# RicoFio/disentangle_mlp

Measured on AMD Instinct MI355X. Metric: celeba64_betavaegan_train_images_per_sec, higher is better.
Workload: dtype fp32-equivalent (fp16x3 split of fp32 operands on the f16 MFMA, fp32 accumulate, every convolution and the Linear layers with >= 2^20 weights (vg_gemm_nt_f16x3); the small Linear layers (vendor GEMMs), BatchNorm, losses, Adam in fp32)

## Files before the change

disentangle_mlp_amd/csrc/common.hpp:

```cpp
#pragma once
#include <hip/hip_runtime.h>
#include <stdint.h>

typedef float f32x16 __attribute__((ext_vector_type(16)));
typedef float f32x4 __attribute__((ext_vector_type(4)));

#define VG_WAVE 64

#ifdef VG_TUNING
#define VG_KNOB(type, name, value) type name = value
#else
#define VG_KNOB(type, name, value) constexpr type name = value
#endif

#define VG_CHECK_LAUNCH()                         \
  do {                                            \
    hipError_t e__ = hipGetLastError();           \
    if (e__ != hipSuccess) return (int)e__;       \
  } while (0)

__device__ __forceinline__ f32x16 mfma32(float a, float b, f32x16 c) {
  return __builtin_amdgcn_mfma_f32_32x32x2f32(a, b, c, 0, 0, 0);
}

__device__ __forceinline__ int acc_row(int r, int lane) {
  return (r & 3) + 8 * (r >> 2) + 4 * (lane >> 5);
}

__device__ __forceinline__ float act_slope(float v, float slope) { return v * (v > 0.f ? 1.f : slope); }

typedef __attribute__((ext_vector_type(8))) __bf16 bf16x8;
typedef __attribute__((ext_vector_type(8))) _Float16 f16x8;

#define VG_PLANES_F16_FLAG 0x100

constexpr int VG_PACK_SPARE = 6;
constexpr size_t vg_pack_trailer_units(int nsteps, int planes, int CoutP) {
  return (size_t)(nsteps + VG_PACK_SPARE) * planes * 2 * CoutP;
}

constexpr int VG_STATS_SLOT_DEPTH = 16;

__device__ __forceinline__ unsigned f16_bound_exp(float amax) {
  const unsigned e = (__float_as_uint(amax) >> 23) & 0xffu;
  return min(max(e, 15u), 254u);
}
__device__ __forceinline__ float f16_scale_of(float amax) { return __uint_as_float((268u - f16_bound_exp(amax)) << 23); }
__device__ __forceinline__ float f16_unscale_of(float amax) { return __uint_as_float((f16_bound_exp(amax) - 14u) << 23); }

template <int NP, bool F16>
__device__ __forceinline__ void split_planes16(float* v, f32x4* out) {
  if constexpr (F16) {
    static_assert(NP == 2, "fp16 planes: hi + lo");
    typedef float f32x2 __attribute__((ext_vector_type(2)));
    typedef _Float16 f16x2 __attribute__((ext_vector_type(2)));
    f16x2 hi[4], lo[4];
#pragma unroll
    for (int j = 0; j < 4; ++j) {
      const f32x2 v2 = {v[2 * j], v[2 * j + 1]};
      const f16x2 h = __builtin_convertvector(v2, f16x2);
      hi[j] = h;
      lo[j] = __builtin_convertvector(v2 - __builtin_convertvector(h, f32x2), f16x2);
    }
    struct P4 { f16x2 q[4]; };
    out[0] = __builtin_bit_cast(f32x4, P4{{hi[0], hi[1], hi[2], hi[3]}});
    out[1] = __builtin_bit_cast(f32x4, P4{{lo[0], lo[1], lo[2], lo[3]}});
  } else {
#pragma unroll
    for (int p = 0; p < NP; ++p) {
      bf16x8 q;
#pragma unroll
      for (int j = 0; j < 8; ++j) {
        const __bf16 h = (__bf16)v[j];
        q[j] = h;
        v[j] -= (float)h;
      }
      out[p] = __builtin_bit_cast(f32x4, q);
    }
  }
}

template <bool F16>
__device__ __forceinline__ f32x16 mfma_split16(bf16x8 a, bf16x8 b, f32x16 c) {
  if constexpr (F16)
    return __builtin_amdgcn_mfma_f32_32x32x16_f16(__builtin_bit_cast(f16x8, a), __builtin_bit_cast(f16x8, b), c, 0, 0, 0);
  else
    return __builtin_amdgcn_mfma_f32_32x32x16_bf16(a, b, c, 0, 0, 0);
}

template <typename T>
__device__ __forceinline__ T wave_sum(T v) {
#pragma unroll
  for (int o = 32; o > 0; o >>= 1) v += __shfl_down(v, o, 64);
  return v;
}

template <typename T>
__device__ __forceinline__ T wave_allsum(T v) {
#pragma unroll
  for (int o = 32; o > 0; o >>= 1) v += __shfl_xor(v, o, 64);
  return v;
}

template <int NT, typename T>
__device__ __forceinline__ T block_sum(T v, T* red) {
  v = wave_sum(v);
  const int lane = threadIdx.x & 63, wid = threadIdx.x >> 6;
  __syncthreads();
  if (lane == 0) red[wid] = v;
  __syncthreads();
  T t = 0;
  if (threadIdx.x == 0) {
#pragma unroll
    for (int i = 0; i < NT / 64; ++i) t += red[i];
  }
  return t;
}

__device__ __forceinline__ unsigned abs_bits(float v) { return __float_as_uint(v) & 0x7fffffffu; }

template <int NT>
__device__ __forceinline__ void block_amax_atomic(unsigned m, unsigned* out) {
  __shared__ unsigned amax_red[NT / 64];
#pragma unroll
  for (int o = 32; o > 0; o >>= 1) m = max(m, (unsigned)__shfl_xor((int)m, o, 64));
  const int lane = threadIdx.x & 63, wid = threadIdx.x >> 6;
  if (lane == 0) amax_red[wid] = m;
  __syncthreads();
  if (threadIdx.x == 0) {
#pragma unroll
    for (int i = 1; i < NT / 64; ++i) m = max(m, amax_red[i]);
    if (m > __hip_atomic_load(out, __ATOMIC_RELAXED, __HIP_MEMORY_SCOPE_AGENT)) atomicMax(out, m);
  }
}

__host__ __device__ constexpr int cdiv(int a, int b) { return (a + b - 1) / b; }

int vg_internal_wgrad_reduce(const float* slabs, float* dw, int n, int splits, hipStream_t st, int accumulate = 0);
size_t vg_internal_ring_workspace_bytes(int mode, int B, int Cin, int H, int W, int Cout, int planes);
size_t vg_internal_ring_stats_floats(int mode, int B, int Cin, int H, int W, int Cout, int planes);
int vg_internal_ring_conv(int mode, const float* x, const void* packed, const float* bias, float* y, int B, int Cin, int H,
                          int W, int Cout, int planes, void* workspace, size_t workspace_bytes, const float* in_scale,
                          const float* in_shift, int in_act, float* stats, size_t stats_floats, const float* in_amax,
                          hipStream_t st);
#ifdef VG_TUNING
void vg_internal_ring_set_variant(int v);
void vg_internal_wx_set_th(int th);
#endif
int vg_internal_convT_s1_thin(const float* x, const float* w, const float* bias, float* y, int B, int Cin, int H,
                              int W, int Cout, hipStream_t st);
```

disentangle_mlp_amd/csrc/wgrad_bf16split.hip:

```cpp
#include <algorithm>
#include <vector>

#include "common.hpp"
#include "vaegan_hip.h"

namespace {

constexpr int WTW = 8, WCIT = 5;

struct WXArgs {
  const float* x;
  int B;
  const float* in_scale;
  const float* in_shift;
  float in_slope;
  const bf16x8* gp;
  float* ws;
  int Cin, H, W, Cout, CoP, OH, OW;
  int mtiles, ntiles, tiles_w, tiles_hw, chunks;
  int units, upw;
  unsigned short order[256];
  const float* x_amax;
};

template <int NP, bool F16>
__global__ __launch_bounds__(256) void relayout_gy_kernel(const float* __restrict__ gy, bf16x8* __restrict__ gp,
                                                         int B, int Co, int CoP, int P, const float* __restrict__ g_scale,
                                                         const float* __restrict__ g_shift, float g_slope,
                                                         const float* __restrict__ g_amax) {
  __shared__ float tile[8][32][33];
  const float gsc16 = F16 ? f16_scale_of(*g_amax) : 1.f;
  const int tid = threadIdx.x;
  const int p0 = blockIdx.x * 32, co0 = blockIdx.y * 32;
  const int bg = blockIdx.z >> 1, kb = blockIdx.z & 1;
  if ((P & 3) == 0 && p0 + 32 <= P && ((uintptr_t)gy & 15) == 0) {
    const int co = co0 + (tid >> 3), q4 = (tid & 7) * 4;
    const float sc = (g_scale && co < Co) ? g_scale[co] : 1.f, sh = (g_scale && co < Co) ? g_shift[co] : 0.f;
    f32x4 v[8];
#pragma unroll
    for (int j = 0; j < 8; ++j) {
      const int b = bg * 16 + kb * 8 + j;
      const float* src = gy + ((size_t)min(b, B - 1) * Co + min(co, Co - 1)) * P + p0 + q4;
      v[j] = *reinterpret_cast<const f32x4*>(src);
    }
#pragma unroll
    for (int j = 0; j < 8; ++j) {
      const bool ok = (bg * 16 + kb * 8 + j) < B && co < Co;
#pragma unroll
      for (int e = 0; e < 4; ++e) {
        float t = v[j][e];
        if (g_scale) {
          t = fmaf(t, sc, sh);
          t = act_slope(t, g_slope);
        }
        tile[j][tid >> 3][q4 + e] = ok ? t : 0.f;
      }
    }
  } else {
    const int r = tid >> 5, pl = tid & 31;
#pragma unroll
    for (int j = 0; j < 8; ++j) {
      const int b = bg * 16 + kb * 8 + j;
#pragma unroll
      for (int rr = 0; rr < 4; ++rr) {
        const int co = co0 + r + 8 * rr;
        float v = 0.f;
        if (b < B && co < Co && p0 + pl < P) {
          v = gy[((size_t)b * Co + co) * P + p0 + pl];
          if (g_scale) {
            v = fmaf(v, g_scale[co], g_shift[co]);
            v = act_slope(v, g_slope);
          }
        }
        tile[j][r + 8 * rr][pl] = v;
      }
    }
  }
  __syncthreads();
  const int cc = tid & 31;
#pragma unroll
  for (int k = 0; k < 4; ++k) {
    const int pp = (tid >> 5) + 8 * k;
    if (p0 + pp >= P) continue;
    float v[8];
#pragma unroll
    for (int j = 0; j < 8; ++j) v[j] = F16 ? tile[j][cc][pp] * gsc16 : tile[j][cc][pp];
    f32x4 pl[NP];
    split_planes16<NP, F16>(v, pl);
#pragma unroll
    for (int p = 0; p < NP; ++p)
      gp[((((size_t)bg * P + p0 + pp) * NP + p) * 2 + kb) * CoP + co0 + cc] = __builtin_bit_cast(bf16x8, pl[p]);
  }
}

constexpr int W8NT = 512;

template <int S_, int NP_, int WCO_, int TH_, bool F16_ = false>
struct W8 {
  static constexpr int S = S_, NP = NP_, WCO = WCO_, WN = 8 / WCO_, FP = 4 / WN, TCO = 32 * WCO_;
  static constexpr bool F16 = F16_;
  static constexpr int TH = TH_, NPIX = TH_ * WTW;
  static constexpr int PD = (FP <= 2) ? 7 : 3;
  static constexpr int PH = S * (TH - 1) + 5, PW = S * (WTW - 1) + 5;
  static constexpr int ROWU = PW + ((5 - PW % 16) + 16) % 16;
  static constexpr int CIU = PH * ROWU + ((9 - (PH * ROWU) % 16) + 16) % 16;
  static constexpr int KBU = WCIT * CIU;
  static constexpr int BUFU = 2 * NP * KBU;
  static constexpr int NUNIT = 2 * WCIT * PH * PW;
  static constexpr int NQ = cdiv(NUNIT, W8NT);
  static constexpr int STEP = TH, ST0 = NPIX / 4;
  static_assert(ST0 + 2 * NQ * STEP <= NPIX, "store schedule");
  static_assert(NPIX % (PD + 1) == 0, "gy ring");
  static_assert(2 * BUFU * 16 <= 160 * 1024, "LDS");
};

template <class C>
__global__ __launch_bounds__(W8NT, 2) void conv5x5_wgrad_split8_kernel(WXArgs A) {
  constexpr int S = C::S, PH = C::PH, PW = C::PW, ROWU = C::ROWU, CIU = C::CIU, KBU = C::KBU, NQ = C::NQ;
  constexpr int NP = C::NP, FP = C::FP, BUFU = C::BUFU, PD = C::PD;
  constexpr bool F16 = C::F16;
  __shared__ f32x4 lds[2 * BUFU];
  const float x_scale = F16 ? f16_scale_of(*A.x_amax) : 1.f;
  const int tid = threadIdx.x, lane = tid & 63;
  const int wid = __builtin_amdgcn_readfirstlane(tid >> 6);
  const int kb = lane >> 5, l32 = lane & 31;
  const int wm = wid % C::WCO, wn = wid / C::WCO;
  const int grp = wid >> 2;
  const int wg = A.order[blockIdx.x];
  const int u_begin = wg * A.upw, u_end = min(u_begin + A.upw, A.units);
  const int Cin = A.Cin, Cout = A.Cout, H = A.H, W = A.W, OW = A.OW, CoP = A.CoP;
  const int HW = H * W, P = A.OH * A.OW;
  int m0 = 0, ci0 = 0;

  int desc[NQ];
#pragma unroll
  for (int q = 0; q < NQ; ++q) {
    const int e = tid + q * W8NT;
    const int col = e % PW;
    int t = e / PW;
    const int r = t % PH;
    t /= PH;
    const int ci = t % WCIT, kbs = min(t / WCIT, 1);
    desc[q] = r | (col << 4) | (ci << 9) | (kbs << 12) | ((e < C::NUNIT ? 1 : 0) << 13);
  }
  static_assert(PH <= 16 && PW <= 32 && WCIT <= 8, "descriptor fields");

  auto chunk_pos = [&](int chunk, int& bg, int& oh, int& ow0) {
    bg = chunk / A.tiles_hw;
    const int sp = chunk % A.tiles_hw;
    oh = (sp / A.tiles_w) * C::TH;
    ow0 = (sp % A.tiles_w) * WTW;
  };
  float preg[NQ][8], psc[NQ], psh[NQ];
  unsigned pvalid = 0;
  const size_t chw = (size_t)Cin * HW;
  auto load_patch = [&](int chunk) {
    int bg, oh, ow0;
    chunk_pos(chunk, bg, oh, ow0);
    const int ih0 = S * oh - 2, iw0 = S * ow0 - 2;
    pvalid = 0;
#pragma unroll
    for (int q = 0; q < NQ; ++q) {
      const int d = desc[q];
      const int ih = ih0 + (d & 15), iw = iw0 + ((d >> 4) & 31);
      const int ci = (d >> 9) & 7, kbs = (d >> 12) & 1;
      const bool ok = ih >= 0 && ih < H && iw >= 0 && iw < W && (ci0 + ci) < Cin;
      pvalid |= ok ? (1u << q) : 0u;
      const int cc = min(ci0 + ci, Cin - 1);
      const unsigned off = (unsigned)(cc * HW + min(max(ih, 0), H - 1) * W + min(max(iw, 0), W - 1));
      psc[q] = A.in_scale ? A.in_scale[cc] : 1.f;
      psh[q] = A.in_scale ? A.in_shift[cc] : 0.f;
      const int b0 = bg * 16 + kbs * 8;
#pragma unroll
      for (int j = 0; j < 8; ++j) {
        const float* xb = A.x + (size_t)min(b0 + j, A.B - 1) * chw;
        preg[q][j] = xb[off];
      }
    }
  };
  auto store_unit = [&](int q, int buf, int chunk) {
    const int bgrp = chunk / A.tiles_hw;
    const int d = desc[q];
    const int kbs = (d >> 12) & 1;
    const bool live = (pvalid >> q) & 1u;
    float v[8];
#pragma unroll
    for (int j = 0; j < 8; ++j) {
      float t = fmaf(preg[q][j], psc[q], psh[q]);
      t = act_slope(t, A.in_slope);
      t = F16 ? t * x_scale : t;
      v[j] = (live && (bgrp * 16 + kbs * 8 + j) < A.B) ? t : 0.f;
    }
    f32x4 pl[NP];
    split_planes16<NP, F16>(v, pl);
    const int dst = buf * BUFU + kbs * KBU + ((d >> 9) & 7) * CIU + (d & 15) * ROWU + ((d >> 4) & 31);
    if (d >> 13) {
#pragma unroll
      for (int p = 0; p < NP; ++p) lds[dst + p * 2 * KBU] = pl[p];
    }
  };
  auto store_patch = [&](int buf, int chunk) {
#pragma unroll
    for (int q = 0; q < NQ; ++q) store_unit(q, buf, chunk);
  };
  static_assert(NQ <= 32, "validity mask");

  int base_b[FP];
#pragma unroll
  for (int f = 0; f < FP; ++f) {
    const int n = min((wn * FP + f) * 32 + l32, WCIT * 25 - 1);
    const int ci = n / 25, tap = n % 25;
    base_b[f] = kb * KBU + ci * CIU + (tap / 5) * ROWU + tap % 5;
  }
  const size_t gstep = (size_t)2 * NP * CoP;
  auto pix_off = [&](int k) -> size_t { return (size_t)(k >> 3) * OW + (k & 7); };

  const int u_split = (u_begin / A.chunks + 1) * A.chunks;
  const bool two = u_split < u_end && u_end <= u_split + A.chunks;
  int u = two ? u_split : u_begin, u_lim = u_end, pass = 0, t0 = 0;
  while (true) {
    if (u >= u_lim) {
      if (!two || pass) break;
      pass = 1;
      u = u_begin;
      u_lim = u_split;
      continue;
    }
    const int tile = u / A.chunks, c_begin = u - tile * A.chunks;
    const int c_end = min(A.chunks, c_begin + (u_lim - u));
    u += c_end - c_begin;
    m0 = (tile % A.mtiles) * C::TCO;
    ci0 = (tile / A.mtiles) * WCIT;
    const bf16x8* ga = A.gp + (size_t)kb * CoP + m0 + wm * 32 + l32;

    f32x16 acc[FP];
#pragma unroll
    for (int f = 0; f < FP; ++f)
#pragma unroll
      for (int r = 0; r < 16; ++r) acc[f][r] = 0.f;

    auto chunk_pix = [&](int chunk) -> size_t {
      int bg, oh, ow0;
      chunk_pos(min(chunk, c_end - 1), bg, oh, ow0);
      return (size_t)bg * P + (size_t)oh * OW + ow0;
    };
    bf16x8 av[PD + 1][NP];
    static_assert((PD == 3 || PD == 7) && WTW == 8, "ring indices below assume 4 or 8 sets, 8 pixels per row");
    auto load_a = [&](int set, size_t pix) {
#pragma unroll
      for (int pl = 0; pl < NP; ++pl) av[set][pl] = ga[pix * gstep + (size_t)pl * 2 * CoP];
    };
    const int nch = c_end - c_begin;
    int rot = ((t0 - c_begin) % A.upw + A.upw) % A.upw;
    rot = rot < nch ? rot : 0;
    t0 += nch;
    auto chunk_at = [&](int j) -> int {
      int i = min(j, nch - 1) + rot;
      i -= (i >= nch) ? nch : 0;
      return c_begin + i;
    };
    load_patch(chunk_at(0));
    store_patch(0, chunk_at(0));
    size_t pcur = chunk_pix(chunk_at(0));
#pragma unroll
    for (int t = 0; t < PD; ++t) load_a(t, pcur + pix_off(t));
    __syncthreads();
    for (int j = 0; j < nch; ++j) {
      const int chn = chunk_at(j + 1);
      const int buf = j & 1;
      const bool more = (j + 1) < nch;
      const size_t pnxt = chunk_pix(chn);
#pragma unroll
      for (int t = 0; t < C::NPIX; ++t) {
        load_a((t + PD) & PD, (t + PD < C::NPIX) ? pcur + pix_off(t + PD) : pnxt + pix_off(t + PD - C::NPIX));
        if (t == 0 && more) load_patch(chn);
        bf16x8 bv[FP][NP];
#pragma unroll
        for (int f = 0; f < FP; ++f)
#pragma unroll
          for (int pl = 0; pl < NP; ++pl)
            bv[f][pl] = __builtin_bit_cast(
                bf16x8, lds[buf * BUFU + base_b[f] + S * (t >> 3) * ROWU + S * (t & 7) + pl * 2 * KBU]);
#pragma unroll
        for (int sum = NP - 1; sum >= 0; --sum)
#pragma unroll
          for (int pa = sum; pa >= 0; --pa)
#pragma unroll
            for (int f = 0; f < FP; ++f) acc[f] = mfma_split16<F16>(av[t & PD][pa], bv[f][sum - pa], acc[f]);
        {
          const int rel = t - C::ST0;
          if (rel >= 0 && rel % C::STEP == 0 && rel / C::STEP < 2 * NQ) {
            const int q = (rel / C::STEP) % NQ, g = (rel / C::STEP) / NQ;
            if (more && grp == g) store_unit(q, buf ^ 1, chn);
          }
        }
      }
      __syncthreads();
      pcur = pnxt;
    }

    const int piece = wg - (int)(((long)tile * A.chunks) / A.upw);
    float* wsb = A.ws + (size_t)piece * Cout * Cin * 25;
#pragma unroll
    for (int f = 0; f < FP; ++f) {
      const int n = (wn * FP + f) * 32 + l32;
      const bool nok = n < WCIT * 25 && (ci0 + n / 25) < Cin;
#pragma unroll
      for (int r16 = 0; r16 < 16; ++r16) {
        const int co = m0 + wm * 32 + acc_row(r16, lane);
        if (nok && co < Cout) wsb[((size_t)co * Cin + ci0) * 25 + n] = acc[f][r16];
      }
    }
  }
}

__global__ __launch_bounds__(256) void wx_reduce_kernel(const float* __restrict__ slabs, float* __restrict__ dw, int Cin,
                                                       int tco, int mtiles, int chunks, int upw, unsigned n, int accumulate,
                                                       const float* __restrict__ x_amax, const float* __restrict__ gy_amax) {
  const unsigned e = blockIdx.x * 256u + threadIdx.x;
  if (e >= n) return;
  const float ux = x_amax ? f16_unscale_of(*x_amax) : 1.f, ug = gy_amax ? f16_unscale_of(*gy_amax) : 1.f;
  const int row = Cin * 25, co = e / row, ci = (e - co * row) / 25;
  const long tile = (long)(ci / WCIT) * mtiles + co / tco;
  const int first = (int)((tile * chunks) / upw), last = (int)(((tile + 1) * chunks - 1) / upw);
  const int cnt = last - first + 1;
  float sum = 0.f;
  int p = 0;
  for (; p + 4 <= cnt; p += 4) {
    float v[4];
#pragma unroll
    for (int k = 0; k < 4; ++k) v[k] = slabs[(size_t)(p + k) * n + e];
#pragma unroll
    for (int k = 0; k < 4; ++k) sum += v[k];
  }
  for (; p < cnt; ++p) sum += slabs[(size_t)p * n + e];
  dw[e] = sum * ux * ug + (accumulate ? dw[e] : 0.f);
}

struct XPlan {
  int BG, CoP, OH, OW, wco, th, mtiles, ntiles, tiles_w, tiles_hw, chunks, units, upw, wgs, pieces;
  size_t gp_bytes, slab_bytes;
};

VG_KNOB(int, g_wx_th, 0);

void plan_shares(XPlan& p, int th) {
  p.th = th;
  p.tiles_hw = p.tiles_w * (p.OH / th);
  p.chunks = p.BG * p.tiles_hw;
  p.units = p.mtiles * p.ntiles * p.chunks;
  p.upw = cdiv(p.units, 256);
  p.wgs = cdiv(p.units, p.upw);
}

bool make_xplan(int B, int Cin, int H, int W, int Cout, int S, int planes, XPlan& p) {
  p.OH = (H - 1) / S + 1;
  p.OW = (W - 1) / S + 1;
  if (p.OW % WTW) return false;
  p.BG = cdiv(B, 16);
  p.CoP = (Cout + 127) & ~127;
  p.wco = Cout > 128 ? 8 : 4;
  p.mtiles = cdiv(Cout, 32 * p.wco);
  p.ntiles = cdiv(Cin, WCIT);
  p.tiles_w = p.OW / WTW;
  if ((long)p.mtiles * p.ntiles * p.BG * p.tiles_w * p.OH > 0x3fffffffL) return false;
  int th = (p.OH % 2 == 0) ? 2 : 1;
  if (g_wx_th == 1 || (g_wx_th == 2 && p.OH % 2 == 0)) th = g_wx_th;
  plan_shares(p, th);
  p.pieces = 0;
  for (long t = 0; t < (long)p.mtiles * p.ntiles; ++t) {
    const int first = (int)((t * p.chunks) / p.upw), last = (int)(((t + 1) * p.chunks - 1) / p.upw);
    p.pieces = last - first + 1 > p.pieces ? last - first + 1 : p.pieces;
  }
  p.gp_bytes = (size_t)p.BG * p.OH * p.OW * 2 * planes * p.CoP * 16;
  p.slab_bytes = (size_t)p.pieces * Cout * Cin * 25 * sizeof(float);
  return true;
}

void make_order(const XPlan& p, unsigned short* order) {
  std::vector<int> idx(p.wgs);
  for (int w = 0; w < p.wgs; ++w) idx[w] = w;
  std::stable_sort(idx.begin(), idx.end(), [&](int a, int b) {
    return ((long)a * p.upw) % p.chunks < ((long)b * p.upw) % p.chunks;
  });
  int start[9];
  start[0] = 0;
  for (int k = 0; k < 8; ++k) start[k + 1] = start[k] + (p.wgs - k + 7) / 8;
  for (int b = 0; b < p.wgs; ++b) order[b] = (unsigned short)idx[start[b & 7] + (b >> 3)];
}

template <class C>
int launch_wx(const WXArgs& A, long grid, hipStream_t st) {
  hipLaunchKernelGGL(conv5x5_wgrad_split8_kernel<C>, dim3((unsigned)grid), dim3(W8NT), 0, st, A);
  VG_CHECK_LAUNCH();
  return 0;
}

template <int S, int NP, bool F16 = false>
int launch_wx_by_cout(const WXArgs& A, int wco, int th, long grid, hipStream_t st) {
  if (th == 2) return wco == 8 ? launch_wx<W8<S, NP, 8, 2, F16>>(A, grid, st) : launch_wx<W8<S, NP, 4, 2, F16>>(A, grid, st);
  return wco == 8 ? launch_wx<W8<S, NP, 8, 1, F16>>(A, grid, st) : launch_wx<W8<S, NP, 4, 1, F16>>(A, grid, st);
}

}

#ifdef VG_TUNING
void vg_internal_wx_set_th(int th) { g_wx_th = (th == 1 || th == 2) ? th : 0; }
#endif

extern "C" size_t vg_conv5x5_wgrad_bf16split_workspace_bytes(int B, int Cin, int H, int W, int Cout, int stride,
                                                          int planes) {
  if (B <= 0 || Cin <= 0 || Cout <= 0 || H <= 0 || W <= 0 || (stride != 1 && stride != 2)) return 0;
  if (planes != 2 && planes != 3 && planes != (VG_PLANES_F16_FLAG | 2)) return 0;
  XPlan p;
  if (!make_xplan(B, Cin, H, W, Cout, stride, planes & 0xff, p)) return 0;
  return p.gp_bytes + p.slab_bytes;
}

extern "C" int vg_conv5x5_wgrad_bf16split(const float* x, const float* gy, float* dw, int B, int Cin, int H, int W,
                                       int Cout, int stride, int planes, void* workspace, size_t workspace_bytes,
                                       const float* in_scale, const float* in_shift, int in_act, int affine_on_gy,
                                       const float* x_amax, const float* gy_amax, int accumulate, void* stream) {
  if (!x || !gy || !dw || B <= 0 || Cin <= 0 || Cout <= 0 || H <= 0 || W <= 0) return VG_ERR_BAD_ARG;
  const bool f16 = (planes & VG_PLANES_F16_FLAG) != 0;
  planes &= 0xff;
  if (f16 && (planes != 2 || !x_amax || !gy_amax)) return VG_ERR_BAD_ARG;
  if (!f16) x_amax = gy_amax = nullptr;
  if ((in_scale == nullptr) != (in_shift == nullptr) || in_act < VG_ACT_NONE || in_act > VG_ACT_LRELU) return VG_ERR_BAD_ARG;
  const float slope = (!in_scale || in_act == VG_ACT_NONE) ? 1.f : (in_act == VG_ACT_RELU ? 0.f : 0.2f);
  const float* gsc = affine_on_gy ? in_scale : nullptr;
  const float* gsh = affine_on_gy ? in_shift : nullptr;
  if (affine_on_gy) in_scale = in_shift = nullptr;
  if ((stride != 1 && stride != 2) || (planes != 2 && planes != 3)) return VG_ERR_BAD_ARG;
  XPlan p;
  if (!make_xplan(B, Cin, H, W, Cout, stride, planes, p)) return VG_ERR_BAD_ARG;
  if (!workspace || ((uintptr_t)workspace & 15) || workspace_bytes < p.gp_bytes + p.slab_bytes)
    return VG_ERR_WORKSPACE;
  hipStream_t st = (hipStream_t)stream;
  bf16x8* gp = (bf16x8*)workspace;
  float* slabs = (float*)((char*)workspace + p.gp_bytes);
  const int P = p.OH * p.OW;
  if ((size_t)Cin * H * W * 4 > 0xffffffffUL || p.BG * 2 > 65535 || p.CoP / 32 > 65535) return VG_ERR_BAD_ARG;
  const dim3 gg(cdiv(P, 32), p.CoP / 32, p.BG * 2);
  if (f16) hipLaunchKernelGGL((relayout_gy_kernel<2, true>), gg, dim3(256), 0, st, gy, gp, B, Cout, p.CoP, P, gsc, gsh, slope, gy_amax);
  else if (planes == 2) hipLaunchKernelGGL((relayout_gy_kernel<2, false>), gg, dim3(256), 0, st, gy, gp, B, Cout, p.CoP, P, gsc, gsh, slope, gy_amax);
  else hipLaunchKernelGGL((relayout_gy_kernel<3, false>), gg, dim3(256), 0, st, gy, gp, B, Cout, p.CoP, P, gsc, gsh, slope, gy_amax);
  VG_CHECK_LAUNCH();
  WXArgs A;
  A.x = x; A.B = B; A.gp = gp; A.ws = slabs; A.x_amax = x_amax;
  A.in_scale = in_scale; A.in_shift = in_shift;
  A.in_slope = in_scale ? slope : 1.f;
  A.Cin = Cin; A.H = H; A.W = W; A.Cout = Cout; A.CoP = p.CoP; A.OH = p.OH; A.OW = p.OW;
  A.mtiles = p.mtiles; A.ntiles = p.ntiles; A.tiles_w = p.tiles_w; A.tiles_hw = p.tiles_hw;
  A.chunks = p.chunks; A.units = p.units; A.upw = p.upw;
  make_order(p, A.order);
  const long grid = p.wgs;
  int rc;
  if (f16) rc = (stride == 2) ? launch_wx_by_cout<2, 2, true>(A, p.wco, p.th, grid, st) : launch_wx_by_cout<1, 2, true>(A, p.wco, p.th, grid, st);
  else if (planes == 2) rc = (stride == 2) ? launch_wx_by_cout<2, 2>(A, p.wco, p.th, grid, st) : launch_wx_by_cout<1, 2>(A, p.wco, p.th, grid, st);
  else rc = (stride == 2) ? launch_wx_by_cout<2, 3>(A, p.wco, p.th, grid, st) : launch_wx_by_cout<1, 3>(A, p.wco, p.th, grid, st);
  if (rc) return rc;
  const unsigned n = (unsigned)Cout * Cin * 25;
  hipLaunchKernelGGL(wx_reduce_kernel, dim3(cdiv(n, 256u)), dim3(256), 0, st, slabs, dw, Cin, 32 * p.wco, p.mtiles,
                     p.chunks, p.upw, n, accumulate ? 1 : 0, x_amax, gy_amax);
  VG_CHECK_LAUNCH();
  return 0;
}
```

Measured before the change: 9295.

## Switch weight-gradient conv kernel from 32x32x16 to 16x16x32 MFMA tiles

Rewrites the inner loop of the 5x5 weight-gradient kernel to use 16x16x32 MFMA instructions, with K of 32 spanning two output pixels (pixel pairs) instead of 32x32x16 over single pixels. Each wave now covers its 32 output channels with two 16-row groups and twice as many 16-wide column tiles. The gradient register ring, LDS B-operand addressing, store schedule and accumulator writeback are reworked to match, and B loads are batched in groups of HB. The aim is better MFMA throughput and fewer accumulator registers per instruction. In exchange it adds more A-operand loads per step and more complex LDS indexing.

```diff
diff --git a/disentangle_mlp_amd/csrc/common.hpp b/disentangle_mlp_amd/csrc/common.hpp
--- a/disentangle_mlp_amd/csrc/common.hpp
+++ b/disentangle_mlp_amd/csrc/common.hpp
@@ -88,6 +88,14 @@
     return __builtin_amdgcn_mfma_f32_32x32x16_bf16(a, b, c, 0, 0, 0);
 }
 
+template <bool F16>
+__device__ __forceinline__ f32x4 mfma_split16x32(bf16x8 a, bf16x8 b, f32x4 c) {
+  if constexpr (F16)
+    return __builtin_amdgcn_mfma_f32_16x16x32_f16(__builtin_bit_cast(f16x8, a), __builtin_bit_cast(f16x8, b), c, 0, 0, 0);
+  else
+    return __builtin_amdgcn_mfma_f32_16x16x32_bf16(a, b, c, 0, 0, 0);
+}
+
 template <typename T>
 __device__ __forceinline__ T wave_sum(T v) {
 #pragma unroll
diff --git a/disentangle_mlp_amd/csrc/wgrad_bf16split.hip b/disentangle_mlp_amd/csrc/wgrad_bf16split.hip
--- a/disentangle_mlp_amd/csrc/wgrad_bf16split.hip
+++ b/disentangle_mlp_amd/csrc/wgrad_bf16split.hip
@@ -99,18 +99,20 @@
 struct W8 {
   static constexpr int S = S_, NP = NP_, WCO = WCO_, WN = 8 / WCO_, FP = 4 / WN, TCO = 32 * WCO_;
   static constexpr bool F16 = F16_;
-  static constexpr int TH = TH_, NPIX = TH_ * WTW;
-  static constexpr int PD = (FP <= 2) ? 7 : 3;
+  static constexpr int TH = TH_, NPAIR = TH_ * WTW / 2;
+  static constexpr int PD = (FP <= 2) ? 3 : 1;
+  static constexpr int HB = (NP == 3) ? 2 : 4;
   static constexpr int PH = S * (TH - 1) + 5, PW = S * (WTW - 1) + 5;
   static constexpr int ROWU = PW + ((5 - PW % 16) + 16) % 16;
   static constexpr int CIU = PH * ROWU + ((9 - (PH * ROWU) % 16) + 16) % 16;
-  static constexpr int KBU = WCIT * CIU;
+  static constexpr int KBU = (WCIT * CIU + 15) & ~15;
   static constexpr int BUFU = 2 * NP * KBU;
   static constexpr int NUNIT = 2 * WCIT * PH * PW;
   static constexpr int NQ = cdiv(NUNIT, W8NT);
-  static constexpr int STEP = TH, ST0 = NPIX / 4;
-  static_assert(ST0 + 2 * NQ * STEP <= NPIX, "store schedule");
-  static_assert(NPIX % (PD + 1) == 0, "gy ring");
+  static constexpr int SPP = 2 / TH, ST0 = NPAIR / 4;
+  static_assert(TH == 1 || TH == 2, "store slots per pair");
+  static_assert(ST0 + cdiv(2 * NQ, SPP) <= NPAIR, "store schedule");
+  static_assert(NPAIR % (PD + 1) == 0, "gy ring");
   static_assert(2 * BUFU * 16 <= 160 * 1024, "LDS");
 };
 
@@ -123,7 +125,7 @@
   const float x_scale = F16 ? f16_scale_of(*A.x_amax) : 1.f;
   const int tid = threadIdx.x, lane = tid & 63;
   const int wid = __builtin_amdgcn_readfirstlane(tid >> 6);
-  const int kb = lane >> 5, l32 = lane & 31;
+  const int kb = (lane >> 4) & 1, pq = lane >> 5, l16 = lane & 15;
   const int wm = wid % C::WCO, wn = wid / C::WCO;
   const int grp = wid >> 2;
   const int wg = A.order[blockIdx.x];
@@ -205,15 +207,15 @@
   };
   static_assert(NQ <= 32, "validity mask");
 
-  int base_b[FP];
-#pragma unroll
-  for (int f = 0; f < FP; ++f) {
-    const int n = min((wn * FP + f) * 32 + l32, WCIT * 25 - 1);
+  int base_b[2 * FP];
+#pragma unroll
+  for (int h = 0; h < 2 * FP; ++h) {
+    const int n = min((wn * 2 * FP + h) * 16 + l16, WCIT * 25 - 1);
     const int ci = n / 25, tap = n % 25;
-    base_b[f] = kb * KBU + ci * CIU + (tap / 5) * ROWU + tap % 5;
+    base_b[h] = kb * KBU + ci * CIU + (tap / 5) * ROWU + tap % 5 + S * pq;
   }
   const size_t gstep = (size_t)2 * NP * CoP;
-  auto pix_off = [&](int k) -> size_t { return (size_t)(k >> 3) * OW + (k & 7); };
+  auto pix_off = [&](int k) -> size_t { return (size_t)(k >> 2) * OW + 2 * (k & 3); };
 
   const int u_split = (u_begin / A.chunks + 1) * A.chunks;
   const bool two = u_split < u_end && u_end <= u_split + A.chunks;
@@ -231,24 +233,26 @@
     u += c_end - c_begin;
     m0 = (tile % A.mtiles) * C::TCO;
     ci0 = (tile / A.mtiles) * WCIT;
-    const bf16x8* ga = A.gp + (size_t)kb * CoP + m0 + wm * 32 + l32;
-
-    f32x16 acc[FP];
-#pragma unroll
-    for (int f = 0; f < FP; ++f)
-#pragma unroll
-      for (int r = 0; r < 16; ++r) acc[f][r] = 0.f;
+    const bf16x8* ga = A.gp + (size_t)pq * gstep + (size_t)kb * CoP + m0 + wm * 32 + l16;
+
+    f32x4 acc[2][2 * FP];
+#pragma unroll
+    for (int g = 0; g < 2; ++g)
+#pragma unroll
+      for (int h = 0; h < 2 * FP; ++h) acc[g][h] = f32x4{0.f, 0.f, 0.f, 0.f};
 
     auto chunk_pix = [&](int chunk) -> size_t {
       int bg, oh, ow0;
       chunk_pos(min(chunk, c_end - 1), bg, oh, ow0);
       return (size_t)bg * P + (size_t)oh * OW + ow0;
     };
-    bf16x8 av[PD + 1][NP];
-    static_assert((PD == 3 || PD == 7) && WTW == 8, "ring indices below assume 4 or 8 sets, 8 pixels per row");
+    bf16x8 av[PD + 1][2][NP];
+    static_assert((PD == 1 || PD == 3) && WTW == 8, "ring indices below assume 2 or 4 sets, 4 pairs per row");
     auto load_a = [&](int set, size_t pix) {
 #pragma unroll
-      for (int pl = 0; pl < NP; ++pl) av[set][pl] = ga[pix * gstep + (size_t)pl * 2 * CoP];
+      for (int g = 0; g < 2; ++g)
+#pragma unroll
+        for (int pl = 0; pl < NP; ++pl) av[set][g][pl] = ga[pix * gstep + (size_t)pl * 2 * CoP + g * 16];
     };
     const int nch = c_end - c_begin;
     int rot = ((t0 - c_begin) % A.upw + A.upw) % A.upw;
@@ -271,26 +275,33 @@
       const bool more = (j + 1) < nch;
       const size_t pnxt = chunk_pix(chn);
 #pragma unroll
-      for (int t = 0; t < C::NPIX; ++t) {
-        load_a((t + PD) & PD, (t + PD < C::NPIX) ? pcur + pix_off(t + PD) : pnxt + pix_off(t + PD - C::NPIX));
+      for (int t = 0; t < C::NPAIR; ++t) {
+        load_a((t + PD) & PD, (t + PD < C::NPAIR) ? pcur + pix_off(t + PD) : pnxt + pix_off(t + PD - C::NPAIR));
         if (t == 0 && more) load_patch(chn);
-        bf16x8 bv[FP][NP];
-#pragma unroll
-        for (int f = 0; f < FP; ++f)
-#pragma unroll
-          for (int pl = 0; pl < NP; ++pl)
-            bv[f][pl] = __builtin_bit_cast(
-                bf16x8, lds[buf * BUFU + base_b[f] + S * (t >> 3) * ROWU + S * (t & 7) + pl * 2 * KBU]);
-#pragma unroll
-        for (int sum = NP - 1; sum >= 0; --sum)
-#pragma unroll
-          for (int pa = sum; pa >= 0; --pa)
-#pragma unroll
-            for (int f = 0; f < FP; ++f) acc[f] = mfma_split16<F16>(av[t & PD][pa], bv[f][sum - pa], acc[f]);
-        {
-          const int rel = t - C::ST0;
-          if (rel >= 0 && rel % C::STEP == 0 && rel / C::STEP < 2 * NQ) {
-            const int q = (rel / C::STEP) % NQ, g = (rel / C::STEP) / NQ;
+#pragma unroll
+        for (int h0 = 0; h0 < 2 * FP; h0 += C::HB) {
+          bf16x8 bv[C::HB][NP];
+#pragma unroll
+          for (int h = 0; h < C::HB; ++h)
+#pragma unroll
+            for (int pl = 0; pl < NP; ++pl)
+              bv[h][pl] = __builtin_bit_cast(
+                  bf16x8, lds[buf * BUFU + base_b[h0 + h] + S * (t >> 2) * ROWU + 2 * S * (t & 3) + pl * 2 * KBU]);
+#pragma unroll
+          for (int sum = NP - 1; sum >= 0; --sum)
+#pragma unroll
+            for (int pa = sum; pa >= 0; --pa)
+#pragma unroll
+              for (int g = 0; g < 2; ++g)
+#pragma unroll
+                for (int h = 0; h < C::HB; ++h)
+                  acc[g][h0 + h] = mfma_split16x32<F16>(av[t & PD][g][pa], bv[h][sum - pa], acc[g][h0 + h]);
+        }
+#pragma unroll
+        for (int i = 0; i < C::SPP; ++i) {
+          const int slot = (t - C::ST0) * C::SPP + i;
+          if (slot >= 0 && slot < 2 * NQ) {
+            const int q = slot % NQ, g = slot / NQ;
             if (more && grp == g) store_unit(q, buf ^ 1, chn);
           }
         }
@@ -302,14 +313,16 @@
     const int piece = wg - (int)(((long)tile * A.chunks) / A.upw);
     float* wsb = A.ws + (size_t)piece * Cout * Cin * 25;
 #pragma unroll
-    for (int f = 0; f < FP; ++f) {
-      const int n = (wn * FP + f) * 32 + l32;
+    for (int h = 0; h < 2 * FP; ++h) {
+      const int n = (wn * 2 * FP + h) * 16 + l16;
       const bool nok = n < WCIT * 25 && (ci0 + n / 25) < Cin;
 #pragma unroll
-      for (int r16 = 0; r16 < 16; ++r16) {
-        const int co = m0 + wm * 32 + acc_row(r16, lane);
-        if (nok && co < Cout) wsb[((size_t)co * Cin + ci0) * 25 + n] = acc[f][r16];
-      }
+      for (int g = 0; g < 2; ++g)
+#pragma unroll
+        for (int r = 0; r < 4; ++r) {
+          const int co = m0 + wm * 32 + g * 16 + 4 * (lane >> 4) + r;
+          if (nok && co < Cout) wsb[((size_t)co * Cin + ci0) * 25 + n] = acc[g][h][r];
+        }
     }
   }
 }
```

After: 9283. No clear change (-0.1%).
